# Distributed-EPFL/at2-node

Measured on AMD Instinct MI355X. Metric: ed25519 verifies/sec (node), higher is better.
Workload: dtype int32; 1 GPU; BASELINE config 2: 1M signed transfers per GPU (100-byte M), dalek-1.x verify; records_per_gpu=1048576, msg_len=100, policy=dalek, senders=distinct, sender_cache=0, sender_comb=False, parallelism=index-shard x1

## Files before the change

### at2-node_amd/csrc/at2v_cpu.cpp

```cpp
#include <sched.h>

#include <algorithm>
#include <atomic>
#include <condition_variable>
#include <cstddef>
#include <cstdint>
#include <cstdio>
#include <cstdlib>
#include <cstring>
#include <mutex>
#include <new>
#include <thread>
#include <vector>

#include "../../include/at2v.h"
#include "at2v_cpu.h"
#include "at2v_fe_fu.h"
#include "at2v_verify.h"
#include "at2v_verify_fu.h"

namespace {

using namespace at2v;

struct CpuTabP {
  gu_cached e[9];
  int pending = 0;
  gu_p3 parked;
  void store(int i, const gu_cached& c) { e[i] = c; }
  void park(const gu_p3& p) { parked = p; }
  void unpark(gu_p3& p) const { p = parked; }
  void prefetch(int i) { pending = i; }
  void load_prefetched(gu_cached& c) const { c = e[pending]; }
};

struct CpuTabB {
  const gu_niels* t;
  mutable int pending = 0;
  void prefetch(int e) const { pending = e; }
  void load_prefetched(gu_niels& n) const { n = t[pending]; }
};

struct CpuTabB8 {
  void load(int i, ge_niels& n) const {
    const int32_t* p = &AT2V_BTAB[i * AT2V_BTAB_WORDS];
    for (int k = 0; k < 10; ++k) {
      n.ypx.v[k] = p[k];
      n.ymx.v[k] = p[10 + k];
      n.xy2d.v[k] = p[20 + k];
    }
  }
};

void build_fixed_range(gu_niels* out, size_t lo, size_t hi, int w, const ge_niels& p1) {
  const size_t N = hi - lo;
  std::vector<ge_p3> P(N);
  {
    uint32_t s[8] = {0, 0, 0, 0, 0, 0, 0, 0};
    s[w] = (uint32_t)lo;
    ge_p2 q;
    ge_scalarmult_base(q, s, CpuTabB8());
    ge_p1p1 r;
    ge_p3 z;
    ge_p3_identity(z);
    ge_niels nq;
    if (lo == 0) {
      P[0] = z;
    } else {
      ge_p2_to_niels(nq, q);
      ge_madd(r, z, nq);
      ge_p1p1_to_p3(P[0], r);
    }
  }
  for (size_t j = 1; j < N; ++j) {
    ge_p1p1 r;
    ge_madd(r, P[j - 1], p1);
    ge_p1p1_to_p3(P[j], r);
  }
  std::vector<fe> pre(N);
  pre[0] = P[0].Z;
  for (size_t j = 1; j < N; ++j) fe_mul(pre[j], pre[j - 1], P[j].Z);
  fe inv;
  fe_invert(inv, pre[N - 1]);
  for (size_t j = N; j-- > 0;) {
    fe zi;
    if (j > 0) {
      fe_mul(zi, inv, pre[j - 1]);
      fe_mul(inv, inv, P[j].Z);
    } else {
      zi = inv;
    }
    fe x, y;
    fe_mul(x, P[j].X, zi);
    fe_mul(y, P[j].Y, zi);
    ge_niels n;
    fe_add(n.ypx, y, x);
    fe_carry32(n.ypx);
    fe_sub(n.ymx, y, x);
    fe_carry32(n.ymx);
    fe_mul(n.xy2d, x, y);
    fe_mul(n.xy2d, n.xy2d, FE_D2);
    niels_fe_to_fu(out[lo + j], n);
  }
}

std::vector<gu_niels> build_fixed_table(int w) {
  const size_t N = (1u << 15) + 1;
  std::vector<gu_niels> out(N);
  uint32_t s1[8] = {0, 0, 0, 0, 0, 0, 0, 0};
  s1[w] = 1;
  ge_p2 q;
  ge_scalarmult_base(q, s1, CpuTabB8());
  ge_niels p1;
  ge_p2_to_niels(p1, q);
  unsigned T = std::thread::hardware_concurrency();
  T = T < 1 ? 1 : T > 16 ? 16 : T;
  std::vector<std::thread> th;
  for (unsigned t = 0; t < T; ++t) {
    const size_t lo = N * t / T, hi = N * (t + 1) / T;
    if (hi > lo) th.emplace_back(build_fixed_range, out.data(), lo, hi, w, p1);
  }
  for (auto& x : th) x.join();
  return out;
}

struct FixedTables {
  std::vector<gu_niels> b0, b1;
};

const FixedTables& fixed_tables() {
  static FixedTables t;
  static std::once_flag once;
  std::call_once(once, [] {
    t.b0 = build_fixed_table(0);
    t.b1 = build_fixed_table(4);
  });
  return t;
}

void le_words(uint32_t w[8], const uint8_t* b) {
  for (int i = 0; i < 8; ++i)
    w[i] = (uint32_t)b[4 * i] | ((uint32_t)b[4 * i + 1] << 8) | ((uint32_t)b[4 * i + 2] << 16) |
           ((uint32_t)b[4 * i + 3] << 24);
}

int verify_record(const uint8_t* pk, const uint8_t* sig, const uint8_t* msg, uint32_t n, int policy) {
  uint32_t R[8], S[8], A[8];
  le_words(R, sig);
  le_words(S, sig + 32);
  le_words(A, pk);
  auto msgword = [&](uint32_t j) -> uint32_t {
    uint32_t v = 0;
    for (uint32_t b = 0; b < 4; ++b)
      if (4 * j + b < n) v |= (uint32_t)msg[4 * j + b] << (8 * b);
    return v;
  };
  const FixedTables& ft = fixed_tables();
  CpuTabP ta, tr;
  const CpuTabB tb0{ft.b0.data()}, tb1{ft.b1.data()};
  auto one = [](int v) { return v; };
  return verify_half_fu(R, A, S, n, msgword, policy, ta, tr, tb0, tb1, one);
}

}

namespace at2v {

unsigned usable_cpus() {
  unsigned n = 0;
#if defined(__linux__)
  cpu_set_t set;
  CPU_ZERO(&set);
  if (sched_getaffinity(0, sizeof set, &set) == 0) n = (unsigned)CPU_COUNT(&set);
#endif
  if (n == 0) n = std::thread::hardware_concurrency();
  if (n == 0) n = 1;
  long long quota = -1, period = 0;
  if (FILE* f = std::fopen("/sys/fs/cgroup/cpu.max", "r")) {
    char q[32] = {0};
    if (std::fscanf(f, "%31s %lld", q, &period) == 2 && std::strcmp(q, "max") != 0) quota = std::atoll(q);
    std::fclose(f);
  } else if (FILE* g = std::fopen("/sys/fs/cgroup/cpu/cpu.cfs_quota_us", "r")) {
    if (std::fscanf(g, "%lld", &quota) != 1) quota = -1;
    std::fclose(g);
    if (FILE* h = std::fopen("/sys/fs/cgroup/cpu/cpu.cfs_period_us", "r")) {
      if (std::fscanf(h, "%lld", &period) != 1) period = 0;
      std::fclose(h);
    }
  }
  if (quota > 0 && period > 0) {
    const unsigned c = (unsigned)((quota + period - 1) / period);
    if (c >= 1 && c < n) n = c;
  }
  return n;
}

struct CpuPool {
  std::vector<std::thread> workers;
  std::mutex m;
  std::condition_variable cv_job, cv_done;
  std::mutex call;
  uint64_t gen = 0;
  bool stop = false;
  size_t busy = 0;
  size_t nchunks = 0;
  std::atomic<size_t> next{0};
  void (*body)(void*, size_t) = nullptr;
  void* arg = nullptr;

  void work() {
    for (size_t c; (c = next.fetch_add(1, std::memory_order_relaxed)) < nchunks;) body(arg, c);
  }
  void worker() {
    uint64_t seen = 0;
    std::unique_lock<std::mutex> lk(m);
    for (;;) {
      cv_job.wait(lk, [&] { return stop || gen != seen; });
      if (stop) return;
      seen = gen;
      lk.unlock();
      work();
      lk.lock();
      if (--busy == 0) cv_done.notify_all();
    }
  }
  void run(size_t chunks, void (*fn)(void*, size_t), void* a) {
    if (chunks == 0) return;
    std::lock_guard<std::mutex> one(call);
    {
      std::lock_guard<std::mutex> lk(m);
      nchunks = chunks;
      next.store(0, std::memory_order_relaxed);
      body = fn;
      arg = a;
      busy = workers.size();
      ++gen;
    }
    cv_job.notify_all();
    work();
    std::unique_lock<std::mutex> lk(m);
    cv_done.wait(lk, [&] { return busy == 0; });
  }
};

namespace {
CpuPool* pool_create(unsigned threads, bool tables) {
  if (threads == 0) threads = usable_cpus();
  if (threads > 1024) threads = 1024;
  CpuPool* p = new (std::nothrow) CpuPool;
  if (!p) return nullptr;
  if (tables) (void)fixed_tables();
  try {
    for (unsigned t = 1; t < threads; ++t) p->workers.emplace_back([p] { p->worker(); });
  } catch (...) {
  }
  return p;
}
}

CpuPool* cpu_pool_create(unsigned threads) { return pool_create(threads, true); }

CpuPool* copy_pool_create(unsigned threads) { return pool_create(threads, false); }

void pool_run(CpuPool* p, size_t chunks, void (*fn)(void*, size_t), void* arg) { p->run(chunks, fn, arg); }

void cpu_pool_destroy(CpuPool* p) {
  if (!p) return;
  {
    std::lock_guard<std::mutex> lk(p->m);
    p->stop = true;
  }
  p->cv_job.notify_all();
  for (auto& t : p->workers) t.join();
  delete p;
}

unsigned cpu_pool_threads(const CpuPool* p) { return p ? (unsigned)p->workers.size() + 1 : 0; }

namespace {
struct BatchJob {
  const uint8_t *pk, *sig, *msg;
  const uint32_t* off;
  size_t n;
  int policy;
  uint32_t* verdicts;
};
void batch_chunk(void* a, size_t c) {
  const BatchJob& j = *static_cast<const BatchJob*>(a);
  const size_t lo = 64 * c, hi = std::min(j.n, lo + 64);
  uint32_t w[2] = {0, 0};
  for (size_t i = lo; i < hi; ++i) {
    const int ok = verify_record(j.pk + 32 * i, j.sig + 64 * i, j.msg + j.off[i], j.off[i + 1] - j.off[i], j.policy);
    w[(i - lo) >> 5] |= (uint32_t)(ok == 1) << (i & 31);
  }
  j.verdicts[2 * c] = w[0];
  if (2 * c + 1 < (j.n + 31) / 32) j.verdicts[2 * c + 1] = w[1];
}
struct DecodeJob {
  const uint8_t* pts;
  size_t n;
  uint32_t* words;
};
void decode_chunk(void* a, size_t c) {
  const DecodeJob& j = *static_cast<const DecodeJob*>(a);
  const size_t lo = 64 * c, hi = std::min(j.n, lo + 64);
  uint32_t w[2] = {0, 0};
  for (size_t i = lo; i < hi; ++i) {
    uint32_t A[8];
    le_words(A, j.pts + 32 * i);
    gu_p3 P;
    w[(i - lo) >> 5] |= (uint32_t)(gu_frombytes(P, A) & 1) << (i & 31);
  }
  j.words[2 * c] = w[0];
  if (2 * c + 1 < (j.n + 31) / 32) j.words[2 * c + 1] = w[1];
}
}

void cpu_verify_batch(CpuPool* p, const uint8_t* pk, const uint8_t* sig, const uint8_t* msg, const uint32_t* msg_off,
                      size_t n, int policy, uint32_t* verdicts) {
  BatchJob j{pk, sig, msg, msg_off, n, policy, verdicts};
  p->run((n + 63) / 64, batch_chunk, &j);
}

void cpu_decode_points(CpuPool* p, const uint8_t* pts, size_t n, uint32_t* valid_words) {
  DecodeJob j{pts, n, valid_words};
  p->run((n + 63) / 64, decode_chunk, &j);
}

}

extern "C" int at2v_verify_one_policy(const uint8_t pk[32], const uint8_t sig[64], const uint8_t* msg, size_t len,
                                      int policy) {
  if (!pk || !sig || (!msg && len) || len >= (1ull << 31)) return AT2V_E_INVALID;
  if (policy != AT2V_POLICY_DALEK_V1 && policy != AT2V_POLICY_LIBSODIUM_1_0_18) return AT2V_E_INVALID;
  return verify_record(pk, sig, msg, (uint32_t)len, policy);
}

extern "C" int at2v_verify_one(const uint8_t pk[32], const uint8_t sig[64], const uint8_t* msg, size_t len) {
  return at2v_verify_one_policy(pk, sig, msg, len, AT2V_POLICY_DALEK_V1);
}
```

### at2-node_amd/csrc/at2v_cpu.h

```cpp
#pragma once
#include <cstddef>
#include <cstdint>

namespace at2v {

struct CpuPool;

unsigned usable_cpus();

CpuPool* cpu_pool_create(unsigned threads);
void cpu_pool_destroy(CpuPool* p);
unsigned cpu_pool_threads(const CpuPool* p);

CpuPool* copy_pool_create(unsigned threads);
void pool_run(CpuPool* p, size_t chunks, void (*fn)(void*, size_t), void* arg);

void cpu_verify_batch(CpuPool* p, const uint8_t* pk, const uint8_t* sig, const uint8_t* msg, const uint32_t* msg_off,
                      size_t n, int policy, uint32_t* verdicts);

void cpu_decode_points(CpuPool* p, const uint8_t* pts, size_t n, uint32_t* valid_words);

}
```

### at2-node_amd/csrc/at2v_kern_tables.h

```cpp
#pragma once
#include <hip/hip_runtime.h>

#include "at2v_comb.h"
#include "at2v_verify.h"
#include "at2v_verify_fu.h"
#include "at2v_fe_fu.h"

namespace at2v {

constexpr int kBlock = 512;
constexpr int kWavesPerBlock = kBlock / 64;
constexpr int kVerifyWavesPerSimd = 2;
static_assert(kBlock == 512, "pacing pairs waves w and w^4 of an 8-wave workgroup");
constexpr size_t kCtlBytes(int grid) { return 64 + (size_t)grid * kWavesPerBlock * 64; }
constexpr int kBWin = 16;
constexpr int kIdentShared = 1;
constexpr int kTabAGranules = (9 - kIdentShared) * 10;
constexpr int kLaneGranules = 2 * kTabAGranules;
constexpr int kNumBtabs = 2;
constexpr size_t kScratchPerWave = (size_t)kLaneGranules * 64 * 16;

#define AT2V_UNIFORM(x) __builtin_amdgcn_readfirstlane(x)


// ... 22 lines not shown
  const uint32_t hl = (i[0] >> 26) | ((i[1] >> 26) << 6) | ((i[2] >> 26) << 12) | ((i[3] >> 25) << 18) |
                      ((i[4] >> 26) << 25) | (p5 << 31);
  const uint32_t hh = (p5 >> 1) | ((i[6] >> 26) << 6) | ((i[7] >> 25) << 12);
  f.v[8] = hl & m26;
  f.v[9] = ((hl >> 26) | (hh << 6)) & m25;
}

struct DevTabA {
  int4* base;
  int4* stage;
  int lane;
  const int4* ident = nullptr;
#ifdef AT2V_WAIT_PROBE
  mutable unsigned long long waited = 0, lds_waited = 0;
#endif
  template <class Cached>
  __device__ AT2V_INLINE void store(int e, const Cached& c) const {
    static_assert(sizeof(Cached) == 160, "cached point: 40 words");
    if (kIdentShared && e == 0) return;
    const int32_t* w = reinterpret_cast<const int32_t*>(&c);
    uint32_t pw[32];
#pragma unroll
    for (int k = 0; k < 4; ++k) {
      fu x;
#pragma unroll
      for (int q = 0; q < 10; ++q) x.v[q] = (uint32_t)w[10 * k + q];
      fu_carry(x);
      fu_pack8(pw + 8 * k, x);
    }
#pragma unroll
    for (int q = 0; q < 8; ++q)
      base[(e - kIdentShared) * 8 + q] =
          make_int4((int)pw[4 * q], (int)pw[4 * q + 1], (int)pw[4 * q + 2], (int)pw[4 * q + 3]);
  }
  template <class P3>
  __device__ AT2V_INLINE void park(const P3& p) const {
    static_assert(sizeof(P3) == 160, "p3 point: 40 words");
    const int32_t* w = reinterpret_cast<const int32_t*>(&p);
#pragma unroll
    for (int q = 0; q < 10; ++q)
      base[(8 - kIdentShared) * 10 + q] = make_int4(w[4 * q], w[4 * q + 1], w[4 * q + 2], w[4 * q + 3]);
  }
  template <class P3>
  __device__ AT2V_INLINE void unpark(P3& p) const {
    int32_t* w = reinterpret_cast<int32_t*>(&p);
    int4 v[10];
#pragma unroll
    for (int q = 0; q < 10; ++q) v[q] = base[(8 - kIdentShared) * 10 + q];
#pragma unroll
    for (int q = 0; q < 10; ++q) {
      w[4 * q] = v[q].x;
      w[4 * q + 1] = v[q].y;
      w[4 * q + 2] = v[q].z;
      w[4 * q + 3] = v[q].w;
    }
  }
  __device__ AT2V_INLINE void prefetch(int e) const {
    const int4* src = (kIdentShared && e == 0) ? ident : base + (e - kIdentShared) * 8;
#pragma unroll
    for (int q = 0; q < 8; ++q)
      __builtin_amdgcn_global_load_lds(reinterpret_cast<const void*>(src + q),
                                       (__attribute__((address_space(3))) void*)(stage + q * 64), 16,
                                       0, 0);
  }
  template <class Cached>
  __device__ AT2V_INLINE void load_prefetched(Cached& c) const {
    static_assert(sizeof(Cached) == 160, "cached point: 40 words");
    AT2V_PROBE(waited, asm volatile("s_waitcnt vmcnt(0)" ::: "memory"));
    uint32_t pw[32];
#pragma unroll
    for (int q = 0; q < 8; ++q) {
      const int4 v = stage[q * 64 + lane];
      pw[4 * q] = (uint32_t)v.x;
      pw[4 * q + 1] = (uint32_t)v.y;
      pw[4 * q + 2] = (uint32_t)v.z;
      pw[4 * q + 3] = (uint32_t)v.w;
    }
    fu* cf = reinterpret_cast<fu*>(&c);
#pragma unroll
    for (int k = 0; k < 4; ++k) fu_unpack8(cf[k], pw + 8 * k);
  }
};

struct LdsTabB {
  const int4* lds;
  __device__ AT2V_INLINE void load(int e, ge_niels& n) const {
    int32_t w[32];
#pragma unroll
    for (int q = 0; q < 8; ++q) {
      const int4 v = lds[e * 8 + q];
      w[4 * q] = v.x;
      w[4 * q + 1] = v.y;
      w[4 * q + 2] = v.z;
      w[4 * q + 3] = v.w;
    }
#pragma unroll
    for (int k = 0; k < 10; ++k) {
      n.ypx.v[k] = w[k];
      n.ymx.v[k] = w[10 + k];
      n.xy2d.v[k] = w[20 + k];
    }
  }
};

constexpr int kBtabEntries = (1 << (kBWin - 1)) + 1;
struct DevTabB {
  const int4* base;
  int4* stage;
  int lane;
#ifdef AT2V_WAIT_PROBE
  mutable unsigned long long waited = 0, lds_waited = 0;
#endif
  __device__ AT2V_INLINE void prefetch(int e) const {
    asm volatile("s_waitcnt lgkmcnt(0)" ::: "memory");
#pragma unroll
    for (int q = 0; q < 8; ++q)
      __builtin_amdgcn_global_load_lds(reinterpret_cast<const void*>(base + e * 8 + q),
                                       (__attribute__((address_space(3))) void*)(stage + q * 64), 16, 0, 0);
  }
  template <class Niels>
  __device__ AT2V_INLINE void load_prefetched(Niels& n) const {
    static_assert(sizeof(Niels) == 120, "Niels point: 30 words");
    AT2V_PROBE(waited, asm volatile("s_waitcnt vmcnt(0)" ::: "memory"));
    int32_t w[32];
#pragma unroll
    for (int q = 0; q < 8; ++q) {
      const int4 v = stage[q * 64 + lane];
      w[4 * q] = v.x;
      w[4 * q + 1] = v.y;
      w[4 * q + 2] = v.z;
      w[4 * q + 3] = v.w;
    }
#pragma unroll
    for (int k = 0; k < 10; ++k) {
      n.ypx.v[k] = w[k];
      n.ymx.v[k] = w[10 + k];
      n.xy2d.v[k] = w[20 + k];
    }
  }
};

#if defined(AT2V_COMB_PROBE) && defined(__HIP_DEVICE_COMPILE__)
#define AT2V_CPROBE(acc, stmt)                                  \
  do {                                                          \
    const unsigned long long t0_ = __builtin_amdgcn_s_memtime(); \
    stmt;                                                       \
    (acc) += __builtin_amdgcn_s_memtime() - t0_;                \
  } while (0)
#else
#define AT2V_CPROBE(acc, stmt) stmt
#endif
#ifdef AT2V_COMB_PROBE
enum {
  kCpAWait,
  kCpBWait,
  kCpStage,
  kCpRecord,
  kCpSha,
  kCpSums,
  kCpFinish,
  kCpBook,
  kCpChunk,
  kCpChunks,
  kCpLds,
  kCpSlot,
  kCpN
// ... 132 lines not shown
```

### at2-node_amd/csrc/at2v_kernels.hip

```cpp
#include <hip/hip_runtime.h>

#include "../../include/at2v.h"
#include "at2v_cache.h"
#include "at2v_comb.h"
#include "at2v_verify.h"
#include "at2v_verify_fu.h"
#include "at2v_fe_fu.h"
#include "at2v_launch.h"
#include "at2v_kern_tables.h"
#include "at2v_kern_cache.h"
#include "at2v_kern_comb.h"
#include "at2v_kern_sign.h"
#include "at2v_kern_btab.h"

namespace at2v {

struct Pace {
  uint32_t* mine;
  const uint32_t* mate;
  uint32_t prog;
  uint32_t mate_prog;
#ifdef AT2V_WAIT_PROBE
  unsigned long long probe[4] = {0, 0, 0, 0};
#endif
// ... 88 lines not shown
  bool dead = false;
  for (uint32_t c = c_first; c < nchunks;) {
    AT2V_PHASE(0);
#ifdef AT2V_WAIT_PROBE
    const unsigned long long t_chunk0 = __builtin_amdgcn_s_memtime();
#endif
    uint32_t i, ii;
    bool act;
    int phit = 0;
    uint32_t pinfo = 0;
    if constexpr (kPart) {
      phit = c < hchunks ? 1 : 0;
      const uint32_t pos = (phit ? c : c - hchunks) * 64 + lane, cnt = phit ? nh : nm;
      const uint32_t pc = pos < cnt ? pos : cnt - 1;
      act = pos < cnt;
      i = ii = (phit ? pp->hidx : pp->midx)[pc];
      if (phit) pinfo = pp->hinfo[pc];
    } else {
      i = c * 64 + lane;
      ii = i < n ? i : n - 1;
      act = i < n;
    }
    int skip = 0;
    if constexpr (kStaged) {
      const uint32_t u0 = (c * 64) >> sp->ushift, u = u0 < sp->nreg - 1 ? u0 : sp->nreg - 1;
      if (u >= known && !dead) known = stage_wait(sp, u + 1, lane, dead);
      skip = u >= known ? 1 : 0;
      const uint8_t* b = arena + sp->at[u];
      const uint32_t rc = u == sp->nreg - 1 ? sp->last_c : 1u << sp->ushift;
      pk = b;
      sig = b + (size_t)rc * 32;
      off = reinterpret_cast<const uint32_t*>(b + (size_t)rc * 96);
      msg = b + (((size_t)rc * 96 + ((size_t)rc + 1) * 4 + 15) & ~(size_t)15);
      msg_total = sp->mb[u];
      ii -= u << sp->ushift;
    }
    uint32_t Rw[8], Sw[8], Aw[8];
    load8(Rw, sig + (size_t)ii * 64);
    load8(Sw, sig + (size_t)ii * 64 + 32);
    load8(Aw, pk + (size_t)ii * 32);
    const uint32_t o0 = off[ii];
    const uint32_t len = off[ii + 1] - o0;
#ifdef AT2V_WAIT_PROBE
    AT2V_PROBE(pace.probe[2], asm volatile("s_waitcnt vmcnt(0)" ::: "memory"));
#endif
    const int msg_fast =
        __builtin_amdgcn_readfirstlane(__all((uint64_t)o0 + len + 8 <= (uint64_t)msg_total) ? 1 : 0);
    const uint32_t* mw = reinterpret_cast<const uint32_t*>(msg) + (o0 >> 2);
    const uint32_t msh = (o0 & 3u) * 8;
    auto msg_unguarded = [=](uint32_t j) -> uint32_t { return __builtin_amdgcn_alignbit(mw[j + 1], mw[j], msh); };
    auto msg_guarded = [=](uint32_t j) -> uint32_t {
      const uint32_t a = o0 + 4 * j;
      const uint32_t a0 = a & ~3u, sh = (a & 3u) * 8;
      const uint32_t lo = load_u32_guarded(msg, a0, msg_total);
      if (sh == 0) return lo;
      const uint32_t hi = load_u32_guarded(msg, a0 + 4, msg_total);
      return __builtin_amdgcn_alignbit(hi, lo, sh);
    };
    auto touched = [] {};
    MsgSplit<decltype(msg_unguarded), decltype(msg_guarded), decltype(touched)> msgword{msg_fast, msg_unguarded,
                                                                                        msg_guarded, touched};
    int good;
    if (kCache) {
      const CacheArgs& cc = *cp;
      int a_ok = 0, u = 0, all_hit;
      if constexpr (kPart) {
        all_hit = phit;
        a_ok = (int)(pinfo & 1u);
        u = (int)(pinfo >> 1);
      } else {
        const int slot = cache_lookup_wave(cc, Aw, lane, i < n);
        const bool hit = cache_hit(cc, slot, Aw, a_ok, u);
        all_hit = __builtin_amdgcn_readfirstlane(__all(hit) ? 1 : 0);
        if (lane == 0) {
          atomicAdd(cc.ctl + kCtlChunks, 1ull);
          if (all_hit) atomicAdd(cc.ctl + kCtlChunkHits, 1ull);
        }
      }
      DevTabA tc{ta};
      if (all_hit) tc.base = cc.payload + (size_t)u * kTabAGranules;
      good = verify_half_fu<true>(Rw, Aw, Sw, len, msgword, policy, tc, tr, tb0, tb1, wmax, pace, all_hit, a_ok) & act;
    } else if (skip) {
      good = 0;
    } else {
      good = verify_half_fu<false>(Rw, Aw, Sw, len, msgword, policy, ta, tr, tb0, tb1, wmax, pace) & act;
    }
    const uint64_t mask = __ballot(good);
#ifdef AT2V_WAIT_PROBE
    AT2V_WAIT_PROBE_SINK(ta.waited + tr.waited, tb0.waited + tb1.waited, pace.probe[0], pace.probe[1],
                         __builtin_amdgcn_s_memtime() - t_chunk0, ta.lds_waited + tr.lds_waited, pace.probe[2]);
    ta.waited = tr.waited = tb0.waited = tb1.waited = ta.lds_waited = tr.lds_waited = tb0.lds_waited = tb1.lds_waited = 0;
    pace.probe[0] = pace.probe[1] = pace.probe[2] = 0;
#endif
    uint32_t ticket = 0;
    if constexpr (kPart) {
      verdict_or(verdicts, i, good, act, lane);
    } else if (lane == 0) {
      verdicts[2 * c] = (uint32_t)mask;
      if (2 * c + 1 < nwords) verdicts[2 * c + 1] = (uint32_t)(mask >> 32);
    }
    if (lane == 0) {
        ticket = atomicAdd(chunk_queue, 1u);
    }
    ticket = __builtin_amdgcn_readfirstlane(ticket);
    c = ticket < nchunks ? nwaves + ticket : nchunks;
    AT2V_PHASE(6);
  }
}

__global__ __launch_bounds__(kBlock, kVerifyWavesPerSimd) void verify_kernel(
    const uint8_t* __restrict__ pk, const uint8_t* __restrict__ sig, const uint8_t* __restrict__ msg,
    uint32_t msg_total, const uint32_t* __restrict__ off, uint32_t n, int policy, uint32_t* __restrict__ verdicts,
    int4* __restrict__ scratch, const int4* __restrict__ btab,
    uint32_t* __restrict__ chunk_queue) {
  __shared__ int4 astage[kWavesPerBlock * 10 * 64];
  __shared__ int4 rstage[kWavesPerBlock * 10 * 64];
  verify_chunks<false>(astage, rstage, pk, sig, msg, msg_total, off, n, policy, verdicts, scratch, btab, chunk_queue,
                       nullptr);
}

__global__ __launch_bounds__(kBlock, kVerifyWavesPerSimd) void verify_kernel_staged(
    const uint8_t* __restrict__ arena, uint32_t n, int policy, uint32_t* __restrict__ verdicts,
    int4* __restrict__ scratch, const int4* __restrict__ btab,
    uint32_t* __restrict__ chunk_queue, StagedArgs sa) {
  __shared__ int4 astage[kWavesPerBlock * 10 * 64];
  __shared__ int4 rstage[kWavesPerBlock * 10 * 64];
  if (threadIdx.x < 64) __builtin_amdgcn_fence(__ATOMIC_ACQUIRE, "");
  __syncthreads();
  verify_chunks<false, false, true>(astage, rstage, arena, arena, arena, 0, nullptr, n, policy, verdicts, scratch, btab,
                                    chunk_queue, nullptr, nullptr, &sa);
}

__global__ __launch_bounds__(kBlock, kVerifyWavesPerSimd) void verify_kernel_cached(
    const uint8_t* __restrict__ pk, const uint8_t* __restrict__ sig, const uint8_t* __restrict__ msg,
    uint32_t msg_total, const uint32_t* __restrict__ off, uint32_t n, int policy, uint32_t* __restrict__ verdicts,
    int4* __restrict__ scratch, const int4* __restrict__ btab,
    uint32_t* __restrict__ chunk_queue, CacheArgs c) {
  __shared__ int4 astage[kWavesPerBlock * 10 * 64];
  __shared__ int4 rstage[kWavesPerBlock * 10 * 64];
  verify_chunks<true>(astage, rstage, pk, sig, msg, msg_total, off, n, policy, verdicts, scratch, btab, chunk_queue,
                      &c);
}

__global__ __launch_bounds__(kBlock, kVerifyWavesPerSimd) void verify_kernel_miss(
    const uint8_t* __restrict__ pk, const uint8_t* __restrict__ sig, const uint8_t* __restrict__ msg,
    uint32_t msg_total, const uint32_t* __restrict__ off, uint32_t n, int policy, uint32_t* __restrict__ verdicts,
    int4* __restrict__ scratch, const int4* __restrict__ btab,
    uint32_t* __restrict__ chunk_queue, PartArgs p) {
  __shared__ int4 astage[kWavesPerBlock * 10 * 64];
  __shared__ int4 rstage[kWavesPerBlock * 10 * 64];
  verify_chunks<false, true>(astage, rstage, pk, sig, msg, msg_total, off, n, policy, verdicts, scratch, btab,
                             chunk_queue, nullptr, &p);
}
__global__ __launch_bounds__(kBlock, kVerifyWavesPerSimd) void verify_kernel_tables_part(
    const uint8_t* __restrict__ pk, const uint8_t* __restrict__ sig, const uint8_t* __restrict__ msg,
    uint32_t msg_total, const uint32_t* __restrict__ off, uint32_t n, int policy, uint32_t* __restrict__ verdicts,
    int4* __restrict__ scratch, const int4* __restrict__ btab,
    uint32_t* __restrict__ chunk_queue, CacheArgs c, PartArgs p) {
  __shared__ int4 astage[kWavesPerBlock * 10 * 64];
  __shared__ int4 rstage[kWavesPerBlock * 10 * 64];
  verify_chunks<true, true>(astage, rstage, pk, sig, msg, msg_total, off, n, policy, verdicts, scratch, btab,
                            chunk_queue, &c, &p);
}

constexpr int kPairBlock = 256;
constexpr int kPairWaves = kPairBlock / 64;
// ... 273 lines not shown
```

### at2-node_amd/csrc/at2v_sc.h

```cpp
#pragma once
#include "at2v_fe_base.h"

namespace at2v {

#define AT2V_L_WORDS {0x5cf5d3edu, 0x5812631au, 0xa2f79cd6u, 0x14def9deu, 0u, 0u, 0u, 0x10000000u}

AT2V_HD AT2V_INLINE int sc_is_canonical(const uint32_t s[8]) {
  const uint32_t l[8] = AT2V_L_WORDS;
  uint64_t borrow = 0;
#pragma unroll
  for (int i = 0; i < 8; ++i) {
    uint64_t d = (uint64_t)s[i] - l[i] - borrow;
    borrow = (d >> 63) & 1;
  }
  return (int)borrow;
}

AT2V_HD AT2V_INLINE void sc_cond_sub_l9(uint32_t r[9]) {
  const uint32_t l[8] = AT2V_L_WORDS;
  uint32_t t[9];
  uint64_t borrow = 0;
#pragma unroll
  for (int i = 0; i < 9; ++i) {
    uint64_t d = (uint64_t)r[i] - (i < 8 ? l[i] : 0u) - borrow;
// ... 5 lines not shown
  for (int i = 0; i < 9; ++i) r[i] = ge ? t[i] : r[i];
}

AT2V_HD AT2V_INLINE void sc_reduce512(uint32_t k[8], const uint32_t x[16]) {
  const uint32_t mu[9] = {0x0a2c131bu, 0xed9ce5a3u, 0x086329a7u, 0x2106215du, 0xffffffebu,
                          0xffffffffu, 0xffffffffu, 0xffffffffu, 0x0000000fu};
  const uint32_t l[8] = AT2V_L_WORDS;
  uint32_t q2[18];
#pragma unroll
  for (int i = 0; i < 18; ++i) q2[i] = 0;
#pragma unroll
  for (int i = 0; i < 9; ++i) {
    uint64_t carry = 0;
#pragma unroll
    for (int j = 0; j < 9; ++j) {
      uint64_t t = (uint64_t)x[7 + i] * mu[j] + q2[i + j] + carry;
      q2[i + j] = (uint32_t)t;
      carry = t >> 32;
    }
    q2[i + 9] = (uint32_t)carry;
  }
  uint32_t r2[9];
#pragma unroll
  for (int i = 0; i < 9; ++i) r2[i] = 0;
#pragma unroll
  for (int i = 0; i < 9; ++i) {
    uint64_t carry = 0;
#pragma unroll
    for (int j = 0; j < 8; ++j) {
      if (i + j < 9) {
        uint64_t t = (uint64_t)q2[9 + i] * l[j] + r2[i + j] + carry;
        r2[i + j] = (uint32_t)t;
        carry = t >> 32;
      }
    }
    if (i + 8 < 9) r2[i + 8] = (uint32_t)carry;
  }
  uint32_t r[9];
  uint64_t borrow = 0;
#pragma unroll
  for (int i = 0; i < 9; ++i) {
    uint64_t d = (uint64_t)x[i] - r2[i] - borrow;
    r[i] = (uint32_t)d;
    borrow = (d >> 63) & 1;
  }
  sc_cond_sub_l9(r);
  sc_cond_sub_l9(r);
#pragma unroll
  for (int i = 0; i < 8; ++i) k[i] = r[i];
}

AT2V_HD AT2V_INLINE void sc_recode4(uint32_t out[8], const uint32_t s[8]) {
  int carry = 0;
#pragma unroll
  for (int j = 0; j < 8; ++j) {
    uint32_t w = 0;
#pragma unroll
    for (int m = 0; m < 8; ++m) {
      int d = (int)((s[j] >> (4 * m)) & 15) + carry;
      carry = (d + 8) >> 4;
      d -= carry << 4;
      w |= (uint32_t)(d + 8) << (4 * m);
    }
    out[j] = w;
  }
}

AT2V_HD AT2V_INLINE void sc_recode4_hi8(uint32_t out[8], const uint32_t s[8]) {
  int carry = 0;
#pragma unroll
  for (int j = 0; j < 8; ++j) {
    uint32_t w = 0;
#pragma unroll
    for (int m = 0; m < 8; ++m) {
      int d = (int)((s[j] >> (4 * m)) & 15) + carry;
      carry = (d + 7) >> 4;
      d -= carry << 4;
      w |= (uint32_t)(d + 7) << (4 * m);
    }
    out[j] = w;
  }
}

AT2V_HD AT2V_INLINE void sc_recode8(uint32_t out[8], const uint32_t s[8]) {
  int carry = 0;
#pragma unroll
  for (int j = 0; j < 8; ++j) {
    uint32_t w = 0;
#pragma unroll
    for (int m = 0; m < 4; ++m) {
      int d = (int)((s[j] >> (8 * m)) & 255) + carry;
      carry = (d + 128) >> 8;
      d -= carry << 8;
      w |= (uint32_t)(d + 128) << (8 * m);
    }
    out[j] = w;
  }
}

AT2V_HD AT2V_INLINE void sc_recode16(uint32_t out[8], const uint32_t s[8]) {
  int carry = 0;
#pragma unroll
  for (int j = 0; j < 8; ++j) {
    uint32_t w = 0;
#pragma unroll
    for (int m = 0; m < 2; ++m) {
      int d = (int)((s[j] >> (16 * m)) & 0xffff) + carry;
      carry = (d + 0x8000) >> 16;
      d -= carry << 16;
      w |= (uint32_t)(d + 0x8000) << (16 * m);
    }
    out[j] = w;
  }
}

template <int WB>
struct ScWin {
  static constexpr int ND = (254 + WB - 1) / WB;
};
template <int WB>
AT2V_HD AT2V_INLINE void sc_recode_w(uint32_t out[ScWin<WB>::ND], const uint32_t s[8]) {
  constexpr int ND = ScWin<WB>::ND;
  int carry = 0;
#pragma unroll
  for (int j = 0; j < ND; ++j) {
    const int bit = WB * j, k = bit >> 5, sh = bit & 31;
    uint32_t raw = k < 8 ? (s[k] >> sh) : 0u;
    if (sh && k + 1 < 8) raw |= s[k + 1] << (32 - sh);
    raw &= (1u << WB) - 1u;
    int d = (int)raw + carry;
    carry = (d + (1 << (WB - 1))) >> WB;
    d -= carry << WB;
    out[j] = (uint32_t)(d + (1 << (WB - 1)));
  }
}

}
```

### at2-node_amd/csrc/at2v_verify_fu.h

```cpp
#pragma once
#include "at2v_comb.h"
#include "at2v_gu.h"
#include "at2v_verify.h"

namespace at2v {

#ifndef AT2V_PARK_POINTS
#define AT2V_PARK_POINTS 0
#endif
#ifndef AT2V_DECODE_X2
#define AT2V_DECODE_X2 0
#endif
#ifndef AT2V_TABLES_X2
#define AT2V_TABLES_X2 0
#endif
#ifndef AT2V_TABLES_EARLY
#define AT2V_TABLES_EARLY 0
#endif
#ifndef AT2V_DECODE_LATE
#define AT2V_DECODE_LATE 0
#endif

#ifndef AT2V_DECODE_LOOP
#define AT2V_DECODE_LOOP 0
// ... 240 lines not shown
    tr.prefetch(dr < 0 ? -dr : dr);
    gu_p3_identity(R3);
    ta.load_prefetched(ca);
    gu_cached_cneg(ca, da < 0);
    gu_add(tt, R3, ca);
    gu_p1p1_to_p3(R3, tt);
    tr.load_prefetched(ca);
    gu_cached_cneg(ca, (dr < 0) ^ rflip);
    gu_add(tt, R3, ca);
    gu_p1p1_to_p2(R2, tt);
  }
#ifndef AT2V_DIGIT_AHEAD
#define AT2V_DIGIT_AHEAD 1
#endif
#if AT2V_DIGIT_AHEAD
  uint32_t wa = sel8(c0d, (nw - 2) >> 3), wr = sel8(c1d, (nw - 2) >> 3);
#endif
  for (int i = nw - 2; i >= 0; --i) {
    const bool bwin = (i & 3) == 0 && i < 32;
    int e0 = 0, e1 = 0;
#if AT2V_DIGIT_AHEAD
    int da, dr;
    AT2V_PROBE(pace.probe[0], {
      da = (int)((wa >> (4 * (i & 7))) & 15) - 7;
      dr = (int)((wr >> (4 * (i & 7))) & 15) - 7;
#if defined(__HIP_DEVICE_COMPILE__)
      asm volatile("" ::"v"(da), "v"(dr) : "memory");
#endif
    });
    pace.window();
    wa = sel8(c0d, (i - 1) >> 3);
    wr = sel8(c1d, (i - 1) >> 3);
    const uint32_t wt0 = sel8(td, i >> 3);
    const uint32_t wt1 = sel8(td, 4 + (i >> 3));
#else
    pace.window();
    const int da = digit4(c0d, i), dr = digit4(c1d, i);
#endif
    ta.prefetch(da < 0 ? -da : da);
    tr.prefetch(dr < 0 ? -dr : dr);
    for (int r = 0; r < 3; ++r) {
      gu_p2_dbl(tt, R2);
      gu_p1p1_to_p2(R2, tt);
    }
    gu_p2_dbl(tt, R2);
    gu_p1p1_to_p3(R3, tt);
    AT2V_PROBE(pace.probe[1], pace.mid());
    if (bwin) {
#if AT2V_DIGIT_AHEAD
      e0 = (1 << 15) - (int)((wt0 >> (16 * ((i >> 2) & 1))) & 0xffff);
      e1 = (1 << 15) - (int)((wt1 >> (16 * ((i >> 2) & 1))) & 0xffff);
#else
      e0 = (1 << 15) - (int)((sel8(td, i >> 3) >> (16 * ((i >> 2) & 1))) & 0xffff);
      e1 = (1 << 15) - (int)((sel8(td, 4 + (i >> 3)) >> (16 * ((i >> 2) & 1))) & 0xffff);
#endif
    }
    ta.load_prefetched(ca);
    if (bwin) tb0.prefetch(e0 < 0 ? -e0 : e0);
    gu_cached_cneg(ca, da < 0);
    gu_add(tt, R3, ca);
    gu_p1p1_to_p3(R3, tt);
    tr.load_prefetched(ca);
    if (bwin) tb1.prefetch(e1 < 0 ? -e1 : e1);
    gu_cached_cneg(ca, (dr < 0) ^ rflip);
    gu_add(tt, R3, ca);
    if (bwin) {
      gu_p1p1_to_p3(R3, tt);
      tb0.load_prefetched(nb);
      gu_niels_cneg(nb, e0 < 0);
      gu_madd(tt, R3, nb);
      gu_p1p1_to_p3(R3, tt);
      tb1.load_prefetched(nb);
      gu_niels_cneg(nb, e1 < 0);
      gu_madd(tt, R3, nb);
    }
    gu_p1p1_to_p2(R2, tt);
  }
  AT2V_PHASE(4);
  fu d;
  fu_sub(d, R2.Y, R2.Z, FU_KC);
  return ok & fu_iszero(R2.X) & fu_iszero(d);
}

template <class TabP, class TabB, class MsgWord, class WaveMax>
AT2V_HD AT2V_INLINE int verify_pair_part(int side, const uint32_t Rw[8], const uint32_t Aw[8], const uint32_t Sw[8],
                                         uint32_t len, MsgWord msgword, int policy, TabP& tp, const TabB& tb,
                                         WaveMax wave_max, gu_p3& out) {
  int ok;
  gu_p3 P;
  if (side == 0) {
    ok = sc_is_canonical(Sw);
    if (policy == POLICY_LIBSODIUM_1_0_18) {
      ok &= !enc_small_order(Rw);
      ok &= enc_y_canonical(Aw) & !enc_small_order(Aw);
    }
  } else {
    ok = enc_y_canonical(Rw);
  }
  ok &= gu_frombytes(P, side ? Rw : Aw);
  if (side) ok &= !(fu_iszero(P.X) & (int)(Rw[7] >> 31));
  AT2V_PHASE(1);
  uint32_t k[8];
  {
    uint32_t pre[16];
#pragma unroll
    for (int i = 0; i < 8; ++i) {
      pre[i] = Rw[i];
      pre[8 + i] = Aw[i];
    }
    uint64_t h[8];
    sha512_msg<16>(h, pre, len, msgword);
    uint32_t hw[16];
    sha512_digest_words(hw, h);
    sc_reduce512(k, hw);
  }
  AT2V_PHASE(5);
  HalfScalars hs;
  lattice_reduce(hs, k);
  AT2V_PHASE(7);
  uint32_t t[8];
  sc_mul_signed(t, hs, Sw);
  uint32_t cd[8], td[8];
  sc_recode4_hi8(cd, side ? hs.c1 : hs.c0);
  sc_recode16(td, t);
  ok &= hs.bits <= 255;
  const int nw_lane = hs.bits <= 255 ? hs.bits / 4 + 1 : 0;
  int nw = wave_max(nw_lane);
  nw = nw < 30 ? 30 : nw;
  AT2V_PHASE(2);
  if (side && hs.c1_neg) {
    fu_neg(P.X, P.X, FU_KC);
    fu_carry(P.X);
    fu_neg(P.T, P.T, FU_KC);
    fu_carry(P.T);
  }
  build_a_table_from(P, tp);
  AT2V_PHASE(3);
  gu_p2 R2;
  gu_p3 R3;
  gu_p1p1 tt;
  gu_cached ca;
  gu_niels nb;
  auto digit4 = [](const uint32_t d[8], int i) -> int { return (int)((sel8(d, i >> 3) >> (4 * (i & 7))) & 15) - 7; };
  {
    const int d = digit4(cd, nw - 1);
    tp.prefetch(d < 0 ? -d : d);
    gu_p3_identity(R3);
    tp.load_prefetched(ca);
    gu_cached_cneg(ca, d < 0);
    gu_add(tt, R3, ca);
    gu_p1p1_to_p2(R2, tt);
  }
  for (int i = nw - 2; i >= 0; --i) {
    const int d = digit4(cd, i);
    tp.prefetch(d < 0 ? -d : d);
    for (int r = 0; r < 3; ++r) {
      gu_p2_dbl(tt, R2);
      gu_p1p1_to_p2(R2, tt);
    }
    gu_p2_dbl(tt, R2);
    gu_p1p1_to_p3(R3, tt);
    const bool bwin = (i & 3) == 0 && i < 32;
    int e = 0;
    if (bwin)
      e = (1 << 15) - (int)((sel8(td, (side ? 4 : 0) + (i >> 3)) >> (16 * ((i >> 2) & 1))) & 0xffff);
    tp.load_prefetched(ca);
// ... 144 lines not shown
```

Baseline: 107.3 million verifies/s.

## Use joint 2-bit Straus table for half-scalar A/R multiexponentiation

Replaces the separate per-point window tables for A and R in the half-size verify with a single joint table of 12 combinations of A and R, indexed by a 2-bit signed recoding of both half scalars. Each step does two doublings and one cached add per digit pair instead of separate adds for each point, while the base-point comb adds stay interleaved. The aim is fewer point additions per verify and a smaller per-lane table. In exchange it costs more doublings per bit processed relative to wider windows, a table build with several extra point ops, and double-buffered LDS staging for the table loads. A CPU reference path is added to check correctness.

```diff
diff --git a/at2-node_amd/csrc/at2v_cpu.cpp b/at2-node_amd/csrc/at2v_cpu.cpp
--- a/at2-node_amd/csrc/at2v_cpu.cpp
+++ b/at2-node_amd/csrc/at2v_cpu.cpp
@@ -32,6 +32,14 @@
   void unpark(gu_p3& p) const { p = parked; }
   void prefetch(int i) { pending = i; }
   void load_prefetched(gu_cached& c) const { c = e[pending]; }
+};
+
+struct CpuTabJ {
+  gu_cached e[kJointEntries];
+  int pending[2] = {0, 0};
+  void store(int i, const gu_cached& c) { e[i] = c; }
+  void prefetch(int st, int i, bool) { pending[st] = i; }
+  void load_prefetched(int st, gu_cached& c) const { c = e[pending[st]]; }
 };
 
 struct CpuTabB {
@@ -144,7 +152,8 @@
            ((uint32_t)b[4 * i + 3] << 24);
 }
 
-int verify_record(const uint8_t* pk, const uint8_t* sig, const uint8_t* msg, uint32_t n, int policy) {
+int verify_record(const uint8_t* pk, const uint8_t* sig, const uint8_t* msg, uint32_t n, int policy,
+                  bool joint = false) {
   uint32_t R[8], S[8], A[8];
   le_words(R, sig);
   le_words(S, sig + 32);
@@ -159,6 +168,10 @@
   CpuTabP ta, tr;
   const CpuTabB tb0{ft.b0.data()}, tb1{ft.b1.data()};
   auto one = [](int v) { return v; };
+  if (joint) {
+    CpuTabJ tj;
+    return verify_half_fu_joint(R, A, S, n, msgword, policy, tj, tb0, tb1, one);
+  }
   return verify_half_fu(R, A, S, n, msgword, policy, ta, tr, tb0, tb1, one);
 }
 
@@ -277,6 +290,10 @@
 
 unsigned cpu_pool_threads(const CpuPool* p) { return p ? (unsigned)p->workers.size() + 1 : 0; }
 
+int cpu_verify_one_joint(const uint8_t pk[32], const uint8_t sig[64], const uint8_t* msg, uint32_t len, int policy) {
+  return verify_record(pk, sig, msg, len, policy, true);
+}
+
 namespace {
 struct BatchJob {
   const uint8_t *pk, *sig, *msg;
diff --git a/at2-node_amd/csrc/at2v_cpu.h b/at2-node_amd/csrc/at2v_cpu.h
--- a/at2-node_amd/csrc/at2v_cpu.h
+++ b/at2-node_amd/csrc/at2v_cpu.h
@@ -20,4 +20,6 @@
 
 void cpu_decode_points(CpuPool* p, const uint8_t* pts, size_t n, uint32_t* valid_words);
 
+int cpu_verify_one_joint(const uint8_t pk[32], const uint8_t sig[64], const uint8_t* msg, uint32_t len, int policy);
+
 }
diff --git a/at2-node_amd/csrc/at2v_kern_tables.h b/at2-node_amd/csrc/at2v_kern_tables.h
--- a/at2-node_amd/csrc/at2v_kern_tables.h
+++ b/at2-node_amd/csrc/at2v_kern_tables.h
@@ -128,6 +128,45 @@
   }
 };
 
+constexpr int kJointGranules = (kJointEntries - kIdentShared) * 8;
+static_assert(kJointGranules <= kLaneGranules, "the joint table fits the lane slot");
+struct DevTabJ {
+  DevTabA t;
+  int stage1;
+  __device__ AT2V_INLINE int4* stage_of(int st) const { return t.stage + (st ? stage1 : 0); }
+  template <class Cached>
+  __device__ AT2V_INLINE void store(int e, const Cached& c) const {
+    t.store(e, c);
+  }
+  __device__ AT2V_INLINE void prefetch(int st, int e, bool stage_just_read) const {
+    if (stage_just_read) asm volatile("s_waitcnt lgkmcnt(0)" ::: "memory");
+    const int4* src = (kIdentShared && e == 0) ? t.ident : t.base + (e - kIdentShared) * 8;
+    int4* const stg = stage_of(st);
+#pragma unroll
+    for (int q = 0; q < 8; ++q)
+      __builtin_amdgcn_global_load_lds(reinterpret_cast<const void*>(src + q),
+                                       (__attribute__((address_space(3))) void*)(stg + q * 64), 16, 0, 0);
+  }
+  template <class Cached>
+  __device__ AT2V_INLINE void load_prefetched(int st, Cached& c) const {
+    static_assert(sizeof(Cached) == 160, "cached point: 40 words");
+    AT2V_PROBE(t.waited, asm volatile("s_waitcnt vmcnt(0)" ::: "memory"));
+    int4* const stg = stage_of(st);
+    uint32_t pw[32];
+#pragma unroll
+    for (int q = 0; q < 8; ++q) {
+      const int4 v = stg[q * 64 + t.lane];
+      pw[4 * q] = (uint32_t)v.x;
+      pw[4 * q + 1] = (uint32_t)v.y;
+      pw[4 * q + 2] = (uint32_t)v.z;
+      pw[4 * q + 3] = (uint32_t)v.w;
+    }
+    fu* cf = reinterpret_cast<fu*>(&c);
+#pragma unroll
+    for (int k = 0; k < 4; ++k) fu_unpack8(cf[k], pw + 8 * k);
+  }
+};
+
 struct LdsTabB {
   const int4* lds;
   __device__ AT2V_INLINE void load(int e, ge_niels& n) const {
diff --git a/at2-node_amd/csrc/at2v_kernels.hip b/at2-node_amd/csrc/at2v_kernels.hip
--- a/at2-node_amd/csrc/at2v_kernels.hip
+++ b/at2-node_amd/csrc/at2v_kernels.hip
@@ -194,6 +194,9 @@
       good = verify_half_fu<true>(Rw, Aw, Sw, len, msgword, policy, tc, tr, tb0, tb1, wmax, pace, all_hit, a_ok) & act;
     } else if (skip) {
       good = 0;
+    } else if constexpr (!kCache && !kPart && !kStaged) {
+      DevTabJ tj{ta, (int)(tr.stage - ta.stage)};
+      good = verify_half_fu_joint(Rw, Aw, Sw, len, msgword, policy, tj, tb0, tb1, wmax, pace) & act;
     } else {
       good = verify_half_fu<false>(Rw, Aw, Sw, len, msgword, policy, ta, tr, tb0, tb1, wmax, pace) & act;
     }
diff --git a/at2-node_amd/csrc/at2v_sc.h b/at2-node_amd/csrc/at2v_sc.h
--- a/at2-node_amd/csrc/at2v_sc.h
+++ b/at2-node_amd/csrc/at2v_sc.h
@@ -111,6 +111,25 @@
   }
 }
 
+AT2V_HD AT2V_INLINE int sc_recode2(uint32_t out[8], const uint32_t s[8]) {
+  uint64_t c = 0;
+  int nd = 0;
+#pragma unroll
+  for (int j = 0; j < 8; ++j) {
+    c += (uint64_t)s[j] + 0x55555555u;
+    out[j] = (uint32_t)c;
+    c >>= 32;
+    const uint32_t x = out[j] ^ 0x55555555u;
+    if (x) nd = 16 * j + (33 - __builtin_clz(x)) / 2;
+  }
+  return c ? 129 : nd;
+}
+
+AT2V_HD AT2V_INLINE int sc_recode2_joint(uint32_t d0[8], uint32_t d1[8], const uint32_t c0[8], const uint32_t c1[8]) {
+  const int n0 = sc_recode2(d0, c0), n1 = sc_recode2(d1, c1);
+  return n0 > n1 ? n0 : n1;
+}
+
 AT2V_HD AT2V_INLINE void sc_recode8(uint32_t out[8], const uint32_t s[8]) {
   int carry = 0;
 #pragma unroll
diff --git a/at2-node_amd/csrc/at2v_verify_fu.h b/at2-node_amd/csrc/at2v_verify_fu.h
--- a/at2-node_amd/csrc/at2v_verify_fu.h
+++ b/at2-node_amd/csrc/at2v_verify_fu.h
@@ -346,6 +346,222 @@
   return ok & fu_iszero(R2.X) & fu_iszero(d);
 }
 
+enum {
+  kJtA = 1, kJtR, kJtApR, kJtAmR, kJt2A, kJt2R, kJt2ApR, kJtAp2R, kJt2Ap2R, kJt2AmR, kJt2RmA, kJointEntries
+};
+
+constexpr uint64_t joint_idx_table() {
+  const int e[16] = {kJtApR,  kJtR, kJtAmR, kJt2AmR,
+                     kJtA,    0,    kJtA,   kJt2A,
+                     kJtAmR,  kJtR, kJtApR, kJt2ApR,
+                     kJt2RmA, kJt2R, kJtAp2R, kJt2Ap2R};
+  uint64_t t = 0;
+  for (int k = 0; k < 16; ++k) t |= (uint64_t)e[k] << (4 * k);
+  return t;
+}
+constexpr uint64_t kJointIdx = joint_idx_table();
+constexpr uint32_t kJointNeg = 1u << 0 | 1u << 1 | 1u << 4 | 1u << 8;
+
+template <class TabJ>
+AT2V_HD AT2V_INLINE void build_joint_table(const gu_p3& A, const gu_p3& R, TabJ& tj) {
+  gu_cached c;
+  gu_p1p1 s;
+  gu_p3 Q, D;
+  gu_p2 q2;
+  gu_niels nA, nR, nn;
+  gu_cached_identity(c);
+  tj.store(0, c);
+  auto niels_of = [](gu_niels& n, const gu_cached& cc) {
+    n.ypx = cc.YpX;
+    fu_carry(n.ypx);
+    n.ymx = cc.YmX;
+    fu_carry(n.ymx);
+    n.xy2d = cc.T2d;
+  };
+  auto put = [&](int e, const gu_p3& P) {
+    gu_p3_to_cached(c, P);
+    tj.store(e, c);
+  };
+  gu_p3_to_cached(c, A);
+  tj.store(kJtA, c);
+  niels_of(nA, c);
+  gu_p3_to_cached(c, R);
+  tj.store(kJtR, c);
+  niels_of(nR, c);
+  gu_madd(s, A, nR);
+  gu_p1p1_to_p3(Q, s);
+  put(kJtApR, Q);
+  gu_p3_to_p2(q2, Q);
+  gu_p2_dbl(s, q2);
+  gu_p1p1_to_p3(Q, s);
+  put(kJt2Ap2R, Q);
+  nn = nR;
+  gu_niels_cneg(nn, 1);
+  gu_madd(s, A, nn);
+  gu_p1p1_to_p3(Q, s);
+  put(kJtAmR, Q);
+  gu_p3_to_p2(q2, A);
+  gu_p2_dbl(s, q2);
+  gu_p1p1_to_p3(D, s);
+  put(kJt2A, D);
+  gu_madd(s, D, nR);
+  gu_p1p1_to_p3(Q, s);
+  put(kJt2ApR, Q);
+  gu_madd(s, D, nn);
+  gu_p1p1_to_p3(Q, s);
+  put(kJt2AmR, Q);
+  gu_p3_to_p2(q2, R);
+  gu_p2_dbl(s, q2);
+  gu_p1p1_to_p3(D, s);
+  put(kJt2R, D);
+  gu_madd(s, D, nA);
+  gu_p1p1_to_p3(Q, s);
+  put(kJtAp2R, Q);
+  gu_niels_cneg(nA, 1);
+  gu_madd(s, D, nA);
+  gu_p1p1_to_p3(Q, s);
+  put(kJt2RmA, Q);
+}
+
+template <class TabJ, class TabB0, class TabB1, class MsgWord, class WaveMax, class Pace = NoPace>
+AT2V_HD AT2V_INLINE int verify_half_fu_joint(const uint32_t Rw[8], const uint32_t Aw[8], const uint32_t Sw[8],
+                                             uint32_t len, MsgWord msgword, int policy, TabJ& tj, const TabB0& tb0,
+                                             const TabB1& tb1, WaveMax wave_max, Pace&& pace = Pace()) {
+  int ok = sc_is_canonical(Sw);
+  if (policy == POLICY_LIBSODIUM_1_0_18) {
+    ok &= !enc_small_order(Rw);
+    ok &= enc_y_canonical(Aw) & !enc_small_order(Aw);
+  }
+  gu_p3 A, R;
+  ok &= gu_frombytes(A, Aw);
+  ok &= gu_frombytes(R, Rw);
+  ok &= enc_y_canonical(Rw);
+  ok &= !(fu_iszero(R.X) & (int)(Rw[7] >> 31));
+  AT2V_PHASE(1);
+  pace.mark(10);
+  uint32_t k[8];
+  {
+    uint32_t pre[16];
+#pragma unroll
+    for (int i = 0; i < 8; ++i) {
+      pre[i] = Rw[i];
+      pre[8 + i] = Aw[i];
+    }
+    uint64_t h[8];
+    sha512_msg<16>(h, pre, len, msgword);
+    uint32_t hw[16];
+    sha512_digest_words(hw, h);
+    sc_reduce512(k, hw);
+  }
+  AT2V_PHASE(5);
+  pace.mark(3);
+  HalfScalars hs;
+  lattice_reduce(hs, k);
+  AT2V_PHASE(7);
+  pace.mark(3);
+  uint32_t t[8];
+  sc_mul_signed(t, hs, Sw);
+  uint32_t c0d[8], c1d[8], td[8];
+  const int nd = sc_recode2_joint(c0d, c1d, hs.c0, hs.c1);
+  sc_recode16(td, t);
+  ok &= hs.bits <= 255;
+  const int nw_lane = ok ? nd : 0;
+  int nw = wave_max(nw_lane);
+  constexpr int kNwMin = 58;
+  nw = nw < kNwMin ? kNwMin : nw;
+  AT2V_PHASE(2);
+  pace.mark(1);
+
+  if (hs.c1_neg) {
+    fu_neg(R.X, R.X, FU_KC);
+    fu_carry(R.X);
+    fu_neg(R.T, R.T, FU_KC);
+    fu_carry(R.T);
+  }
+  build_joint_table(A, R, tj);
+  AT2V_PHASE(3);
+  pace.mark(4);
+
+  gu_p2 R2;
+  gu_p3 R3;
+  gu_p1p1 tt;
+  gu_cached ca;
+  gu_niels nb;
+  auto key2 = [](uint32_t wa, uint32_t wr, int i) -> uint32_t {
+    const int sh = 2 * (i & 15);
+    return ((wa >> sh) & 3u) | (((wr >> sh) & 3u) << 2);
+  };
+  auto entry_of = [](uint32_t key) -> int { return (int)((uint32_t)(kJointIdx >> (4 * key)) & 15u); };
+  auto neg_of = [](uint32_t key) -> int { return (int)((kJointNeg >> key) & 1u); };
+  int neg_cur, e_next, neg_next;
+  {
+    const int i = nw - 1;
+    const uint32_t k1 = key2(sel8(c0d, i >> 4), sel8(c1d, i >> 4), i);
+    const uint32_t k0 = key2(sel8(c0d, (i - 1) >> 4), sel8(c1d, (i - 1) >> 4), i - 1);
+    tj.prefetch(i & 1, entry_of(k1), false);
+    tj.prefetch((i - 1) & 1, entry_of(k0), false);
+    neg_cur = neg_of(k0);
+    gu_p3_identity(R3);
+    tj.load_prefetched(i & 1, ca);
+    gu_cached_cneg(ca, neg_of(k1));
+    gu_add(tt, R3, ca);
+    gu_p1p1_to_p2(R2, tt);
+  }
+  uint32_t wa = sel8(c0d, (nw - 3) >> 4), wr = sel8(c1d, (nw - 3) >> 4);
+  for (int i = nw - 2; i >= 0; --i) {
+    const bool bwin = (i & 7) == 0 && i < 64;
+    {
+      const uint32_t kn = key2(wa, wr, i - 1);
+      e_next = entry_of(kn);
+      neg_next = neg_of(kn);
+#if defined(__HIP_DEVICE_COMPILE__)
+      asm volatile("" ::"v"(e_next), "v"(neg_next) : "memory");
+#endif
+    }
+    if (i & 1) pace.window();
+    wa = sel8(c0d, (i - 2) >> 4);
+    wr = sel8(c1d, (i - 2) >> 4);
+    uint32_t wt0 = 0, wt1 = 0;
+    if (bwin) {
+      wt0 = sel8(td, i >> 4);
+      wt1 = sel8(td, 4 + (i >> 4));
+    }
+    gu_p2_dbl(tt, R2);
+    gu_p1p1_to_p2(R2, tt);
+    gu_p2_dbl(tt, R2);
+    gu_p1p1_to_p3(R3, tt);
+    tj.load_prefetched(i & 1, ca);
+    int e0 = 0, e1 = 0;
+    if (bwin) {
+      e0 = (1 << 15) - (int)((wt0 >> (16 * ((i >> 3) & 1))) & 0xffff);
+      e1 = (1 << 15) - (int)((wt1 >> (16 * ((i >> 3) & 1))) & 0xffff);
+      tb0.prefetch(e0 < 0 ? -e0 : e0);
+      tb1.prefetch(e1 < 0 ? -e1 : e1);
+    } else {
+      tj.prefetch((i - 1) & 1, e_next, false);
+    }
+    gu_cached_cneg(ca, neg_cur);
+    gu_add(tt, R3, ca);
+    if (bwin) {
+      gu_p1p1_to_p3(R3, tt);
+      tb0.load_prefetched(nb);
+      gu_niels_cneg(nb, e0 < 0);
+      gu_madd(tt, R3, nb);
+      gu_p1p1_to_p3(R3, tt);
+      tb1.load_prefetched(nb);
+      if (i > 0) tj.prefetch((i - 1) & 1, e_next, true);
+      gu_niels_cneg(nb, e1 < 0);
+      gu_madd(tt, R3, nb);
+    }
+    gu_p1p1_to_p2(R2, tt);
+    neg_cur = neg_next;
+  }
+  AT2V_PHASE(4);
+  fu d;
+  fu_sub(d, R2.Y, R2.Z, FU_KC);
+  return ok & fu_iszero(R2.X) & fu_iszero(d);
+}
+
 template <class TabP, class TabB, class MsgWord, class WaveMax>
 AT2V_HD AT2V_INLINE int verify_pair_part(int side, const uint32_t Rw[8], const uint32_t Aw[8], const uint32_t Sw[8],
                                          uint32_t len, MsgWord msgword, int policy, TabP& tp, const TabB& tb,
```

Measured after the change: 110.3 million verifies/s, median of 6. 2.9% higher.
